# jcjones/ct-mapreduce

Measured on AMD Instinct MI355X. Metric: certificates/sec whole-node + achieved HBM GB/s, 100M-entry synthetic CT batch, higher is better.
Workload: dtype u8

## Files before the change

ct_mapreduce_amd/csrc/ctmr_engine.hip:

```cpp
#include <hip/hip_runtime.h>
#include <dlfcn.h>
#include <rccl/rccl.h>

#include <algorithm>
#include <atomic>
#include <chrono>
#include <condition_variable>
#include <deque>
#include <system_error>
#include <thread>
#include <cmath>
#include <cstdarg>
#include <cstdio>
#include <cstdlib>
#include <cstring>
#include <map>
#include <mutex>
#include <set>
#include <string>
#include <unordered_map>
#include <vector>

#include "host_keys.h"
#include "kernels.h"
// ... 161 lines not shown
  unsigned long long* issuer_counts = nullptr;
  uint32_t epoch = 0;
  bool pairs_dirty = false;
  int known_order = CTMR_KNOWN_ORDER_ANY;
  uint32_t max_issuers = 0;
  uint8_t* d_issuer_valid = nullptr;
  uint32_t* d_canon = nullptr;
  std::vector<IssuerRec> issuers;
  std::unordered_map<std::string, uint32_t> id_to_canon;
  uint8_t* d_idb_der = nullptr;
  size_t idb_cap = 0, idb_used = 0;
  uint64_t* d_idb_off = nullptr;
  uint32_t* d_idb_len = nullptr;
  unsigned long long* d_idb_ht = nullptr;
  uint32_t idb_ht_size = 0;
  std::vector<unsigned long long> h_idb_ht;
  std::unordered_map<std::string, uint32_t> der_to_idx;
  bool auto_register = true;
  int chain0_mode = CTMR_CHAIN0_EXACT;
  bool strict_ext = true;
  bool strict_strings = true;
  bool strict_spki = true;
  bool strict_leaf = true;
  uint64_t meta_precheck_n = 0;
  const uint32_t* meta_precheck_ent = nullptr;
  std::unordered_map<unsigned long long, uint32_t> qh_first;
  std::vector<std::string> pending_issuers;
  unsigned long long* d_pend = nullptr;
  uint32_t* d_unreg = nullptr;
  unsigned long long* d_dcount = nullptr;
  MetaSlot* d_meta_slots = nullptr;
  uint64_t n_meta_slots = 0;
  uint8_t* d_meta_arena = nullptr;
  unsigned long long* d_meta_refs = nullptr;
  uint64_t meta_arena_cap = 0;
  std::vector<uint32_t*> meta_hour_pages;
  uint32_t** d_meta_hour_pages = nullptr;
  unsigned long long* d_mcount = nullptr;
  uint64_t meta_n = 0;
  uint32_t meta_epoch = 0;
  unsigned long long* d_bloom = nullptr;
  uint64_t bloom_words = 0;
  bool bloom_owned = false;
  uint64_t bloom_round_ref0 = ~0ull;
  bool last_meta_valid = false;
  uint64_t last_meta_items = 0;
  bool last_is_view = false;
  size_t last_o_start = 0, last_o_end = 0;
  FilterDev* d_filter = nullptr;
  FilterDev h_filter{};
  DevStats* d_stats = nullptr;
  uint32_t* d_result = nullptr;
  unsigned long long* d_count = nullptr;
  void* d_scratch[28] = {};
  size_t scratch_cap[28] = {};
  RoundCtx rd;
  uint64_t last_n = 0, last_n_new = 0;
  size_t last_o_off = 0, last_o_new = 0;
  hipEvent_t ev[8] = {};
  std::vector<uint64_t> h_rel;
  std::map<std::string, std::set<std::string>> hstore;
  std::map<std::string, int64_t> expiry;
  std::unordered_map<uint32_t, uint64_t> host_issuer_counts;
};

namespace {

enum { SC_RECORDS = 0, SC_SLOTID, SC_BLKNEW, SC_BLKBASE, SC_ENT, SC_STAGE_A, SC_STAGE_B, SC_MISC, SC_PEM, SC_PEMOFF, SC_TMP, SC_VIEW, SC_ISS_A, SC_ISS_B, SC_ISS_C, SC_META, SC_ITEMS,
       SC_XSTAGE, SC_XWCNT, SC_XCNT, SC_XBASE, SC_XSLOT, SC_XL,
       SC_NFX,
       SC_KEYPOS,
       SC_PEMBLK,
       SC_PEMINFO
       };
constexpr uint32_t UNREG_CAP = 16384;

int fail(const ctmr_engine* e, int code, const char* fmt, ...) {
  char buf[512];
  va_list ap;
  va_start(ap, fmt);
  vsnprintf(buf, sizeof buf, fmt, ap);
  va_end(ap);
  if (e) {
    std::lock_guard<std::mutex> g(e->err_mu);
    e->err = buf;
  }
  return code;
}

#define HIPCHK(e, call)                                                                   \
  do {                                                                                    \
    hipError_t _r = (call);                                                               \
    if (_r != hipSuccess)                                                                 \
      return fail(e, _r == hipErrorOutOfMemory ? CTMR_E_NOMEM : CTMR_E_HIP, "%s: %s", #call, \
                  hipGetErrorString(_r));                                                 \
  } while (0)

int ensure(ctmr_engine* e, int which, size_t bytes) {
  if (e->scratch_cap[which] >= bytes) return CTMR_OK;
  if (e->d_scratch[which]) {
    HIPCHK(e, hipStreamSynchronize(e->stream));
    HIPCHK(e, hipFree(e->d_scratch[which]));
    e->d_scratch[which] = nullptr;
    e->scratch_cap[which] = 0;
  }
  size_t cap = bytes + bytes / 8 + 256;
  HIPCHK(e, hipMalloc(&e->d_scratch[which], cap));
  e->scratch_cap[which] = cap;
  return CTMR_OK;
}

struct DevMem {
  void* p = nullptr;
  DevMem() = default;
  DevMem(const DevMem&) = delete;
  DevMem& operator=(const DevMem&) = delete;
  ~DevMem() { if (p) (void)hipFree(p); }
  hipError_t alloc(size_t bytes) {
    if (p) (void)hipFree(p);
    p = nullptr;
    const hipError_t r = hipMalloc(&p, bytes);
    if (r != hipSuccess) {
      (void)hipGetLastError();
      p = nullptr;
    }
    return r;
// ... 332 lines not shown
```

ct_mapreduce_amd/csrc/engine/map.inc:

```

int ctmr_set_filter(ctmr_engine* e, const char* filter, size_t len, int log_expired, int64_t now) {
  if (!e || (len && !filter)) return CTMR_E_INVAL;
  std::lock_guard<std::mutex> g(e->mu);
  HIPCHK(e, hipSetDevice(e->device));
  FilterDev f;
  memset(&f, 0, sizeof f);
  f.active = len != 0;
  f.log_expired = log_expired != 0;
  f.now = now;
  f.strict_spki = e->strict_spki ? 1u : 0u;
  f.strict_strings = e->strict_strings ? 1u : 0u;
  f.strict_ext = e->strict_ext ? 1u : 0u;
  size_t s = 0;
  uint32_t nw = 0;
  for (;;) {
    size_t t = s;
    while (t < len && filter[t] != ',') t++;
    const size_t pl = t - s;
    if (f.n_pieces >= 64 || nw + (pl + 3) / 4 > 1024)
      return fail(e, CTMR_E_INVAL, "issuerCNFilter too large (max 64 pieces / 4096 bytes)");
    f.piece_len[f.n_pieces] = (uint32_t)pl;
    f.piece_word[f.n_pieces] = nw;
    memcpy((uint8_t*)(f.words + nw), filter + s, pl);
    nw += (uint32_t)((pl + 3) / 4);
    f.n_pieces++;
    if (t >= len) break;
    s = t + 1;
  }
  e->h_filter = f;
  return upload_filter(e);
}

static int launch_map(ctmr_engine* e, const uint8_t* d_payload, const uint64_t* d_offsets,
                      const uint32_t* d_issuer_idx, const uint8_t* d_entry_type, uint64_t n,
                      ctmr_record* d_records, bool optimistic_new, const InsertArgs* fuse = nullptr,
                      const uint64_t* d_ends = nullptr, uint64_t limit = 0, int mode = XM_LOCAL,
                      const XchgArgs* xchg = nullptr, uint64_t first = 0) {
  MapArgs ma;
  ma.optimistic_new = optimistic_new ? 1u : 0u;
  ma.ends = d_ends; ma.limit = limit;
  ma.meta_loc = nullptr;
  if (e->cfg.collect_meta) {
    int mr;
    if ((mr = ensure(e, SC_META, (first + n) * 8))) return mr;
    ma.meta_loc = (uint2*)e->d_scratch[SC_META] + first;
    e->meta_n = first + n;
    e->last_meta_valid = false;
  }
  ma.payload = d_payload; ma.offsets = d_offsets; ma.issuer_idx = d_issuer_idx;
  ma.entry_type = d_entry_type; ma.records = d_records; ma.issuer_valid = e->d_issuer_valid;
  ma.filt = e->d_filter; ma.n = n; ma.n_issuers = (uint32_t)e->issuers.size();
  ma.certs_per_tile = 0; ma.lds_bytes = 0;
  ma.keypos = nullptr;
  if (e->strict_spki && n) {
    int kr;
    if ((kr = ensure(e, SC_KEYPOS, (first + n) * 8))) return kr;
    ma.keypos = (unsigned long long*)e->d_scratch[SC_KEYPOS] + first;
  }
  uint32_t variant = e->cfg.map_variant ? e->cfg.map_variant : 15;
  e->meta_precheck_n = 0;
  if (variant == 15 && !fuse) variant = 13;
  const dim3 grid((unsigned)((n + 63) / 64));
#ifdef CTMR_SWEEP
  static const size_t extra_lds = getenv("CTMR_EXTRA_LDS") ? (size_t)atoi(getenv("CTMR_EXTRA_LDS")) : 0;
#else
  constexpr size_t extra_lds = 0;
#endif
  const bool strict = e->strict_strings || e->strict_ext;
  if (variant == 15) {
    MetaCheck mc{};
    XchgArgs xa{};
    if (xchg) xa = *xchg;
    bool meta = false;
    if (e->cfg.collect_meta && e->d_meta_slots) {
      mc.slots = e->d_meta_slots; mc.mask = e->n_meta_slots - 1; mc.arena = e->d_meta_arena;
      mc.hour_pages = e->d_meta_hour_pages; mc.n_hour_pages = e->d_meta_hour_pages ? (uint32_t)e->meta_hour_pages.size() : 0u;
      mc.refs = e->d_meta_refs; mc.n_refs = e->max_issuers;
      mc.enabled = 1;
      meta = true;
      e->meta_precheck_n = first + n;
      e->meta_precheck_ent = fuse->ent - first;
    }
#define CTMR_LAUNCH_FUSED(META, MODE)                                                                                        \
  do {                                                                                                                       \
    if (strict)                                                                                                              \
      hipLaunchKernelGGL((k_map_fused<WIN_CH_STRICT, META, MODE, true>), grid, dim3(64),                                     \
                         WinGeo<WIN_CH_STRICT>::LDS_BYTES + extra_lds, e->stream, ma, *fuse, mc, xa);                        \
    else                                                                                                                     \
      hipLaunchKernelGGL((k_map_fused<WIN_CH_FAST, META, MODE, false>), grid, dim3(64),                                      \
                         WinGeo<WIN_CH_FAST>::LDS_BYTES + extra_lds, e->stream, ma, *fuse, mc, xa);                          \
  } while (0)
    if (mode == XM_OWNER) { if (meta) CTMR_LAUNCH_FUSED(true, XM_OWNER); else CTMR_LAUNCH_FUSED(false, XM_OWNER); }
    else if (mode == XM_BLOOM) { if (meta) CTMR_LAUNCH_FUSED(true, XM_BLOOM); else CTMR_LAUNCH_FUSED(false, XM_BLOOM); }
    else { if (meta) CTMR_LAUNCH_FUSED(true, XM_LOCAL); else CTMR_LAUNCH_FUSED(false, XM_LOCAL); }
#undef CTMR_LAUNCH_FUSED
  } else if (variant == 13) {
    if (strict) hipLaunchKernelGGL((k_map_winc<WIN_CH_STRICT, true>), grid, dim3(64), WinGeo<WIN_CH_STRICT>::LDS_BYTES + extra_lds, e->stream, ma);
    else hipLaunchKernelGGL((k_map_winc<WIN_CH_FAST, false>), grid, dim3(64), WinGeo<WIN_CH_FAST>::LDS_BYTES + extra_lds, e->stream, ma);
#ifdef CTMR_SWEEP
  } else if (variant == 2) {
    hipLaunchKernelGGL(k_map_direct, dim3((unsigned)((n + 255) / 256)), dim3(256), 0, e->stream, ma);
  } else if (variant == 1 && !d_ends) {
    uint32_t C = e->cfg.certs_per_tile ? e->cfg.certs_per_tile : 32;
    if (C > 64) C = 64;
    uint32_t lds = e->cfg.lds_tile_bytes ? e->cfg.lds_tile_bytes : 65536;
    if (lds > 160 * 1024) lds = 160 * 1024;
    ma.certs_per_tile = C; ma.lds_bytes = lds;
    if (!e->tile_attr_set) {
      HIPCHK(e, hipFuncSetAttribute((const void*)k_map_tile, hipFuncAttributeMaxDynamicSharedMemorySize, 160 * 1024));
      e->tile_attr_set = true;
    }
    hipLaunchKernelGGL(k_map_tile, dim3((unsigned)((n + C - 1) / C)), dim3(64), lds, e->stream, ma);
#endif
  } else {
    return fail(e, CTMR_E_INVAL, "map_variant %u is not built into this library", variant);
  }
  return CTMR_OK;
}

static bool round_fused(const ctmr_engine* e) { return e->cfg.map_variant == 0 || e->cfg.map_variant == 15; }

static void round_insert_args(ctmr_engine* e, const RoundCtx& rc, InsertArgs& ia) {
  ia.records = rc.d_records; ia.payload = rc.d_payload; ia.offsets = rc.d_offsets; ia.ends = rc.d_ends; ia.canon = e->d_canon;
  ia.t = e->tbl(); ia.ref0 = rc.ref0; ia.slot_id = (uint32_t*)e->d_scratch[SC_SLOTID];
  ia.ent = (uint32_t*)e->d_scratch[SC_ENT]; ia.n = rc.n; ia.stats = e->d_stats; ia.ord_base = rc.ord_base;
  ia.keypos = (const unsigned long long*)e->d_scratch[SC_KEYPOS]; ia.stage = nullptr; ia.bloom = nullptr; ia.bloom_wmask = 0;
}

static int round_prepare(ctmr_engine* e, RoundCtx& rc) {
  HIPCHK(e, hipSetDevice(e->device));
  e->rd.valid = false;
  const uint64_t n = rc.n;
  if (n >= 0xfffffff0ull) return fail(e, CTMR_E_INVAL, "batch too large (n < 2^32-16)");
  if (((uintptr_t)rc.d_payload & 15) != 0) return fail(e, CTMR_E_INVAL, "payload must be 16-byte aligned");
  int r;
  if (!rc.d_records) {
    if ((r = ensure(e, SC_RECORDS, n * sizeof(ctmr_record)))) return r;
    rc.d_records = (ctmr_record*)e->d_scratch[SC_RECORDS];
  }
  const uint64_t nb = (n + 1023) / 1024;
  if ((r = ensure(e, SC_SLOTID, n * 4))) return r;
  if ((r = ensure(e, SC_ENT, n * 4))) return r;
  if ((r = ensure(e, SC_BLKNEW, nb * 4))) return r;
  if ((r = ensure(e, SC_BLKBASE, nb * 8))) return r;
  if (e->strict_spki && n && (r = ensure(e, SC_KEYPOS, n * 8))) return r;
  if (e->cfg.collect_meta && (r = ensure(e, SC_META, n * 8))) return r;
  if ((r = ensure_capacity(e, n, true))) return r;
  rc.ref0 = e->arena_used;
  e->arena_used += n;
  e->epoch++;
  e->pairs_dirty = true;
  HIPCHK(e, hipMemsetAsync(e->d_stats, 0, 2 * sizeof(DevStats), e->stream));
  const bool fused = round_fused(e);
  if (!fused && rc.mode == XM_OWNER) return fail(e, CTMR_E_INVAL, "the owner-computes exchange needs the fused map kernel (map_variant 0 / 15)");
  if (rc.mode == XM_LOCAL && fused && e->d_bloom) {
    rc.mode = XM_BLOOM;
  }
  if (rc.mode == XM_BLOOM && !e->d_bloom) return fail(e, CTMR_E_INVAL, "ctmr_bloom_config has not been called");
  return CTMR_OK;
}

static int round_launch_range(ctmr_engine* e, RoundCtx& rc, const XchgArgs* xchg, uint64_t lo, uint64_t hi) {
  const uint64_t n = hi - lo;
  if (!n) return CTMR_OK;
  const bool prof = e->cfg.profile != 0;
  int r;
  InsertArgs ia;
  round_insert_args(e, rc, ia);
  ia.records += lo; ia.offsets += lo; ia.slot_id += lo; ia.ent += lo; ia.n = n; ia.ref0 += lo; ia.ord_base += (uint32_t)lo;
  if (ia.ends) ia.ends += lo;
  if (ia.keypos) ia.keypos += lo;
  const bool fused = round_fused(e);
  XchgArgs xa{};
  if (xchg) xa = *xchg;
  if (xa.stage) xa.stage += lo;
  if (xa.wave_cnt) xa.wave_cnt += (lo / 64) * MAX_WORLD;
  if (rc.mode == XM_BLOOM) {
    xa.bloom = e->d_bloom;
    xa.bloom_wmask = e->bloom_words - 1;
  }
  if (prof && lo == 0) HIPCHK(e, hipEventRecord(e->ev[0], e->stream));
  const int kmode = !fused ? XM_LOCAL : (rc.mode == XM_OWNER && rc.world == 1) ? XM_LOCAL : rc.mode;
  if ((r = launch_map(e, rc.d_payload, rc.d_offsets + lo, rc.d_issuer_idx + lo, rc.d_entry_type ? rc.d_entry_type + lo : nullptr, n,
                      rc.d_records + lo, true, fused ? &ia : nullptr, rc.d_ends ? rc.d_ends + lo : nullptr,
                      rc.blob_bytes + CTMR_PAYLOAD_PAD, kmode, &xa, lo)))
    return r;
  if (prof && hi == rc.n) HIPCHK(e, hipEventRecord(e->ev[1], e->stream));
  if (!fused) hipLaunchKernelGGL(k_insert, dim3((unsigned)((n + 255) / 256)), dim3(256), 0, e->stream, ia);
  if (e->strict_spki) {
    ia.stage = (kmode == XM_OWNER) ? xa.stage : nullptr;
    ia.bloom = (rc.mode == XM_BLOOM && fused) ? xa.bloom : nullptr;
    ia.bloom_wmask = xa.bloom_wmask;
    hipLaunchKernelGGL(k_ec_resolve<true>, dim3((unsigned)((n + EC_PER_BLOCK - 1) / EC_PER_BLOCK)), dim3(256), 0, e->stream, ia, rc.d_records + lo);
    hipLaunchKernelGGL(k_ec_resolve<false>, dim3((unsigned)((n + EC_PER_BLOCK - 1) / EC_PER_BLOCK)), dim3(256), 0, e->stream, ia, rc.d_records + lo);
  }
  hipLaunchKernelGGL(k_insert2, dim3((unsigned)((n + INSERT2_PER_BLOCK - 1) / INSERT2_PER_BLOCK)), dim3(256), 0, e->stream, ia, rc.d_records + lo);
  if (!fused && rc.mode == XM_BLOOM)
    hipLaunchKernelGGL(k_bloom_add, dim3((unsigned)((n + 255) / 256)), dim3(256), 0, e->stream, ia, e->d_bloom, e->bloom_words - 1);
  if (prof && hi == rc.n) HIPCHK(e, hipEventRecord(e->ev[2], e->stream));
  return CTMR_OK;
}

static int round_begin(ctmr_engine* e, RoundCtx& rc, const XchgArgs* xchg) {
  int r;
  if ((r = round_prepare(e, rc))) return r;
  return round_launch_range(e, rc, xchg, 0, rc.n);
}

static void round_compact(ctmr_engine* e, const RoundCtx& rc) {
  const uint64_t nb = (rc.n + 1023) / 1024;
  uint32_t* d_blk_new = (uint32_t*)e->d_scratch[SC_BLKNEW];
  uint64_t* d_blk_base = (uint64_t*)e->d_scratch[SC_BLKBASE];
  hipLaunchKernelGGL(k_scan_blocks, dim3(1), dim3(1024), 0, e->stream, d_blk_new, nb, d_blk_base);
  hipLaunchKernelGGL(k_compact, dim3((unsigned)nb), dim3(256), 0, e->stream, (const ctmr_record*)rc.d_records,
                     (const uint32_t*)e->d_scratch[SC_ENT], rc.n, (const uint64_t*)d_blk_base, rc.d_new_idx);
}

static int round_resolve(ctmr_engine* e, RoundCtx& rc, bool compact_now) {
  const bool prof = e->cfg.profile != 0;
  const uint64_t nb = (rc.n + 1023) / 1024;
  ResolveArgs ra;
  ra.ent = (uint32_t*)e->d_scratch[SC_ENT]; ra.issuer_counts = e->issuer_counts; ra.stats = e->d_stats;
  ra.blk_new = (uint32_t*)e->d_scratch[SC_BLKNEW]; ra.n = rc.n;
  hipLaunchKernelGGL(k_resolve, dim3((unsigned)(nb < 512 ? nb : 512)), dim3(1024), 0, e->stream, ra, nb);
  if (prof) HIPCHK(e, hipEventRecord(e->ev[3], e->stream));
  rc.compacted = false;
  if (compact_now && rc.d_new_idx) {
    round_compact(e, rc);
    rc.compacted = true;
  }
  if (prof) HIPCHK(e, hipEventRecord(e->ev[4], e->stream));
  return CTMR_OK;
}

static int round_collect(ctmr_engine* e, RoundCtx& rc) {
  const uint64_t n = rc.n;
  uint32_t* d_ent = (uint32_t*)e->d_scratch[SC_ENT];
  uint32_t* d_blk_new = (uint32_t*)e->d_scratch[SC_BLKNEW];
  DevStats both[2];
  uint64_t ends[2] = {0, rc.blob_bytes};
  HIPCHK(e, hipMemcpyAsync(both, e->d_stats, sizeof both, hipMemcpyDeviceToHost, e->stream));
// ... 184 lines not shown
```

ct_mapreduce_amd/csrc/kernels/reduce.h:

```cpp
#pragma once
#include "keyrec.h"
#include "map.h"

namespace ctmr {

#define AGENT __HIP_MEMORY_SCOPE_AGENT

__device__ __forceinline__ unsigned long long ld_agent(const unsigned long long* p) {
  return __hip_atomic_load(p, __ATOMIC_RELAXED, AGENT);
}
__device__ __forceinline__ void st_agent(unsigned long long* p, unsigned long long v) {
  __hip_atomic_store(p, v, __ATOMIC_RELAXED, AGENT);
}

__device__ __forceinline__ bool cell_equals(const KeyCell* c, unsigned long long meta, const unsigned long long s[5]) {
  bool eq = (ld_agent(&c->meta) & ~CELL_SHADOW) == meta;
#pragma unroll
  for (int k = 0; k < 5; k++) eq = eq && ld_agent(&c->s[k]) == s[k];
  return eq;
}
__device__ __forceinline__ void cell_write(KeyCell* c, unsigned long long meta, const unsigned long long s[5], uint32_t ord) {
  uint4* q = (uint4*)c;
  q[0] = make_uint4((uint32_t)meta, (uint32_t)(meta >> 32), (uint32_t)s[0], (uint32_t)(s[0] >> 32));
  q[1] = make_uint4((uint32_t)s[1], (uint32_t)(s[1] >> 32), (uint32_t)s[2], (uint32_t)(s[2] >> 32));
  q[2] = make_uint4((uint32_t)s[3], (uint32_t)(s[3] >> 32), (uint32_t)s[4], (uint32_t)(s[4] >> 32));
  q[3] = make_uint4(ord, 0u, 0u, 0u);
}

__device__ __forceinline__ uint32_t index_upsert(const Table& t, unsigned long long meta, const unsigned long long s[5],
                                                 unsigned long long my_ref, bool insert, bool* created,
                                                 unsigned long long* holder = nullptr) {
  const unsigned long long h = key_hash(meta, s);
  const unsigned long long mine = idx_word(h, my_ref);
  uint64_t j = h & t.mask;
  *created = false;
  for (uint64_t probes = 0; probes <= t.mask; probes++) {
    unsigned long long w = ld_agent(&t.index[j]);
    if (w == 0ull) {
      if (!insert) return SID_NONE;
      const unsigned long long old = atomicCAS(&t.index[j], 0ull, mine);
      if (old == 0ull) {
        *created = true;
        if (holder) *holder = mine;
        return (uint32_t)j;
      }
      w = old;
    }
    if (w != IDX_TOMB && idx_same_tag(w, h) && cell_equals(t.arena + (w & REF_MASK), meta, s)) {
      if (holder) *holder = w;
      return (uint32_t)j;
    }
    j = probe_next(j, probes, t.mask);
  }
  return SID_FULL;
}

struct InsertArgs {
  const ctmr_record* records;
  const uint8_t* payload;
  const uint64_t* offsets;
  const uint64_t* ends;
  const uint32_t* canon;
  Table t;
  unsigned long long ref0;
  uint32_t* slot_id;
  uint32_t* ent;
  uint64_t n;
  DevStats* stats;
  uint32_t ord_base;
  const unsigned long long* keypos;
  KeyRec32* stage;
  unsigned long long* bloom;
  uint64_t bloom_wmask;
};

enum : uint32_t {
  ES_NONE = 0,
  ES_CLAIMED = 1,
  ES_DEFER = 2,
  ES_DUP = 3,
  ES_HOST = 4,
  ES_FULL = 5,
  ES_REMOTE = 6,
  ES_PENDING = 7
};
constexpr uint32_t ENT_KEY_PENDING = 0x80u;
__device__ __forceinline__ uint32_t ent_pack(uint32_t status, uint32_t state, uint32_t canon) {
  return (status & 7u) | (state << 3) | (canon << 8);
}
__device__ __forceinline__ uint32_t ent_state(uint32_t e) { return (e >> 3) & 7u; }
__device__ __forceinline__ bool ent_is_new(uint32_t e) {
  const uint32_t st = ent_state(e);
  return (st == ES_CLAIMED) | (st == ES_DEFER) | (st == ES_REMOTE);
}
__device__ __forceinline__ void mark_dup(uint32_t* ent, ctmr_record* records, uint32_t loser) {
  ((uint8_t*)(ent + loser))[0] = (uint8_t)(CTMR_ST_PASS | (ES_DUP << 3));
  uint8_t* fl = (uint8_t*)(records + loser) + 1;
  *fl = (uint8_t)(*fl & ~CTMR_FL_WAS_UNKNOWN);
}

__device__ __forceinline__ uint32_t serial_content_off(const GlobalReader& r, uint32_t L) {
  bool ok = true;
  uint32_t tag, cs, ce;
  rd_hdr(r, L, 0, L, ok, tag, cs, ce);
  rd_hdr(r, L, cs, L, ok, tag, cs, ce);
  uint32_t q = cs;
  if ((r.ld4(q) & 0xffu) == 0xa0u) {
    rd_hdr<false>(r, L, q, L, ok, tag, cs, ce);
    rd_hdr(r, L, cs, L, ok, tag, cs, ce);
    q = ce;
  }
  rd_hdr(r, L, q, L, ok, tag, cs, ce);
  return cs;
}

__device__ __forceinline__ void record_key(const InsertArgs& a, uint64_t i, const uint4& r0,
                                           const uint4& r1, unsigned long long s[5]) {
  const uint32_t slen = r0.x >> 16;
  s[0] = (unsigned long long)r0.w | ((unsigned long long)r1.x << 32);
  s[1] = (unsigned long long)r1.y | ((unsigned long long)r1.z << 32);
  s[2] = (unsigned long long)r1.w;
  s[3] = 0;
  s[4] = 0;
  if (slen > 20) {
    uint64_t lo, hi;
    cert_range(a.offsets, a.ends, i, lo, hi);
    GlobalReader g{(const uint32_t*)a.payload, lo};
    const uint32_t so = serial_content_off(g, (uint32_t)(hi - lo));
    uint32_t x[5] = {0, 0, 0, 0, 0};
#pragma unroll
    for (int k = 0; k < 5; k++) {
      const uint32_t pos = 20u + 4u * k;
      if (pos < slen) {
        const uint32_t rem = slen - pos;
        const uint32_t v = g.ld4(so + pos);
        x[k] = rem >= 4 ? v : (v & (0xffffffffu >> (8 * (4 - rem))));
      }
    }
    s[2] |= (unsigned long long)x[0] << 32;
    s[3] = (unsigned long long)x[1] | ((unsigned long long)x[2] << 32);
    s[4] = (unsigned long long)x[3] | ((unsigned long long)x[4] << 32);
  }
}

__device__ __forceinline__ uint32_t insert_probe_h(const InsertArgs& a, uint64_t i, unsigned long long meta,
                                                   const unsigned long long s[5], unsigned long long h) {
  const unsigned long long mine = idx_word(h, a.ref0 + i);
  uint64_t j = h & a.t.mask;
  for (uint64_t probes = 0; probes <= a.t.mask; probes++) {
    const unsigned long long old = atomicCAS(&a.t.index[j], 0ull, mine);
    if (old == 0ull) return ES_CLAIMED;
// ... 27 lines not shown

__device__ __forceinline__ void store_cells_wave(KeyCell* cells, uint64_t n_left, uint4* img, uint32_t lane, bool keyed,
                                                 unsigned long long meta, const unsigned long long s[5], uint32_t ord) {
  uint4* my = img + lane * 4;
  const unsigned long long m = keyed ? meta : 0ull;
  my[0] = make_uint4((uint32_t)m, (uint32_t)(m >> 32), (uint32_t)s[0], (uint32_t)(s[0] >> 32));
  my[1] = make_uint4((uint32_t)s[1], (uint32_t)(s[1] >> 32), (uint32_t)s[2], (uint32_t)(s[2] >> 32));
  my[2] = make_uint4((uint32_t)s[3], (uint32_t)(s[3] >> 32), (uint32_t)s[4], (uint32_t)(s[4] >> 32));
  my[3] = make_uint4(ord, 0u, 0u, 0u);
  __builtin_amdgcn_wave_barrier();
  const uint32_t nvec = n_left >= 64 ? 256u : (uint32_t)n_left * 4u;
  uint4* out = (uint4*)cells;
#pragma unroll
  for (int r = 0; r < 4; r++)
    if (64u * r + lane < nvec) out[64 * r + lane] = img[64 * r + lane];
}

__global__ void __launch_bounds__(256) k_insert(InsertArgs a) {
  __shared__ __attribute__((aligned(16))) uint4 img[4][64 * 4];
  const uint64_t i = (uint64_t)blockIdx.x * 256 + threadIdx.x;
  const uint32_t lane = threadIdx.x & 63, wv = threadIdx.x >> 6;
  uint32_t state = ES_NONE, status = CTMR_ST__COUNT, canon = 0;
  unsigned long long meta = 0ull, s[5] = {0ull, 0ull, 0ull, 0ull, 0ull};
  bool keyed = false;
  if (i < a.n) {
    const uint4* rp = (const uint4*)(a.records + i);
    const uint4 r0 = rp[0];
    status = r0.x & 0xffu;
    const bool pending = ((r0.x >> 8) & FL_KEY_PENDING) != 0u;
    uint32_t fl_out = (r0.x >> 8) & 0xffu & ~FL_KEY_PENDING;
    if (status == CTMR_ST_PASS) {
      canon = a.canon[r0.z];
      const uint4 r1 = rp[1];
      const uint32_t slen = r0.x >> 16;
      if (pending && slen <= CTMR_MAX_SERIAL) {
        state = ES_PENDING;
        record_key(a, i, r0, r1, s);
        meta = key_meta((int32_t)r0.y, canon, slen);
      } else {
        state = insert_probe(a, i, r0, r1, canon, meta, s);
      }
      keyed = slen <= CTMR_MAX_SERIAL;
      if (state != ES_CLAIMED && state != ES_DEFER && state != ES_PENDING) fl_out &= ~(uint32_t)CTMR_FL_WAS_UNKNOWN;
    }
    if (fl_out != ((r0.x >> 8) & 0xffu)) ((uint8_t*)(a.records + i))[1] = (uint8_t)fl_out;
    a.ent[i] = ent_pack(status, state, canon) | (pending ? ENT_KEY_PENDING : 0u);
    const unsigned long long mp = __ballot(pending);
    if (mp && lane == (uint32_t)(__ffsll((long long)mp) - 1) && ld_agent(&a.stats->n_pending) == 0ull) {
      st_agent(&a.stats->n_pending, 1ull);
      st_agent(&a.stats->n_pending_other, 1ull);
    }
  }
  const uint64_t first = (uint64_t)blockIdx.x * 256 + 64u * wv;
  if (first < a.n)
    store_cells_wave(a.t.arena + a.ref0 + first, a.n - first, img[wv], lane, keyed, meta, s, a.ord_base + (uint32_t)i);
}

__device__ __forceinline__ void mark_dup_ord(const InsertArgs& a, ctmr_record* records, uint32_t loser_ord) {
  const uint32_t li = loser_ord - a.ord_base;
  if ((uint64_t)li < a.n) mark_dup(a.ent, records, li);
}

__device__ __forceinline__ bool settle_order(const InsertArgs& a, ctmr_record* records, uint32_t sid, unsigned long long h,
                                             unsigned long long my_ref, uint32_t ord) {
  unsigned long long w = ld_agent(&a.t.index[sid]);
  for (;;) {
    const unsigned long long href = w & REF_MASK;
    if (href == my_ref) return true;
    if (href < a.ref0) return false;
    const uint32_t hord = __hip_atomic_load(&a.t.arena[href].ord, __ATOMIC_RELAXED, AGENT);
    if (hord < ord) return false;
    const unsigned long long old = atomicCAS(&a.t.index[sid], w, idx_word(h, my_ref));
    if (old == w) {
      mark_dup_ord(a, records, hord);
      return true;
    }
    w = old;
  }
}

__device__ __forceinline__ void insert2_one(const InsertArgs& a, ctmr_record* records, uint64_t i, uint32_t e) {
  uint32_t sid = a.slot_id[i];
  const uint4* rp = (const uint4*)(a.records + i);
  const uint4 r0 = rp[0], r1 = rp[1];
  unsigned long long s[5];
  record_key(a, i, r0, r1, s);
  const unsigned long long meta = key_meta((int32_t)r0.y, e >> 8, r0.x >> 16);
  const unsigned long long h = key_hash(meta, s);
  const uint32_t ord = a.ord_base + (uint32_t)i;
  const unsigned long long my_ref = a.ref0 + i;
  const unsigned long long w = ld_agent(&a.t.index[sid]);
  if (!cell_equals(a.t.arena + (w & REF_MASK), meta, s)) {
    bool created;
    unsigned long long holder = 0ull;
    sid = index_upsert(a.t, meta, s, my_ref, true, &created, &holder);
    if (sid == SID_FULL) {
      ((uint8_t*)(a.ent + i))[0] = (uint8_t)(CTMR_ST_PASS | (ES_FULL << 3));
      return;
    }
    if (created) return;
    if ((holder & REF_MASK) < a.ref0) {
      mark_dup(a.ent, records, (uint32_t)i);
      return;
    }
  }
  if (!settle_order(a, records, sid, h, my_ref, ord)) mark_dup(a.ent, records, (uint32_t)i);
}

constexpr uint32_t INSERT2_PER_BLOCK = 1024;
__global__ void __launch_bounds__(256) k_insert2(InsertArgs a, ctmr_record* records) {
  const uint64_t i0 = (uint64_t)blockIdx.x * INSERT2_PER_BLOCK + threadIdx.x * 4u;
  if (i0 >= a.n) return;
  uint32_t e[4] = {0u, 0u, 0u, 0u};
  if (i0 + 4 <= a.n) {
    const uint4 v = *(const uint4*)(a.ent + i0);
    e[0] = v.x; e[1] = v.y; e[2] = v.z; e[3] = v.w;
  } else {
    for (uint32_t k = 0; i0 + k < a.n; k++) e[k] = a.ent[i0 + k];
  }
  uint32_t todo = (ent_state(e[0]) == ES_DEFER ? 1u : 0u) | (ent_state(e[1]) == ES_DEFER ? 2u : 0u) |
                  (ent_state(e[2]) == ES_DEFER ? 4u : 0u) | (ent_state(e[3]) == ES_DEFER ? 8u : 0u);
  while (todo) {
    const uint32_t k = (uint32_t)__builtin_ctz(todo);
    todo &= todo - 1u;
    const uint32_t ek = k == 0u ? e[0] : k == 1u ? e[1] : k == 2u ? e[2] : e[3];
    insert2_one(a, records, i0 + k, ek);
  }
}

template <int WCH, bool META, int MODE, bool STRICT = false>
__global__ void __launch_bounds__(64) k_map_fused(MapArgs a, InsertArgs ia, MetaCheck mc, XchgArgs xa) {
  const uint64_t first = (uint64_t)blockIdx.x * 64;
  const uint32_t lane = threadIdx.x;
  const uint64_t i = first + lane;
  const bool live = i < a.n;
  const uint64_t limit = map_limit(a);
  uint64_t lo = 0, hi = 0;
  if (live) cert_range(a.offsets, a.ends, i, lo, hi);
  EntryIn in{CTMR_NO_ISSUER, 0u, false, false};
  uint32_t canon = 0;
  if (live) {
    in = load_entry_in(a, i);
    canon = in.iss_in_range ? ia.canon[in.iss] : 0u;
  }
  unsigned long long dn_ref = 0, crl_ref = 0;
  const uint32_t* hour_row = nullptr;
  if constexpr (META) {
    if (live && mc.enabled && in.iss_in_range) {
      if (canon < mc.n_refs) {
        dn_ref = mc.refs[canon];
        crl_ref = mc.refs[mc.n_refs + canon];
      }
      if (canon / META_HOUR_PAGE < mc.n_hour_pages)
        hour_row = mc.hour_pages[canon / META_HOUR_PAGE] + (uint64_t)(canon % META_HOUR_PAGE) * (META_HOUR_BITS / 32);
    }
  }
  const WaveBuf wb = wave_buf(a.payload, limit, lo);
  const uint32_t lrel = wave_rel(wb, lo, live);
  const uint32_t w_me = lrel == REL_NONE ? REL_NONE : ((lrel + WinGeo<WCH>::SKIP) & ~3u);
  U16t hd16{0u, 0u, 0u, 0u};
  bool hd_ok = false;
  if constexpr (WinGeo<WCH>::SKIP != 0u) {
    hd_ok = live & (lo + 16ull <= limit);
    hd16 = *(const U16t*)(a.payload + (hd_ok ? lo : 0ull));
  }
  coop_fill<WCH, false>(wb, w_me, lane);
  uint4 o0 = make_uint4(0, 0, 0, 0), o1 = o0;
  unsigned long long kmeta = 0ull, ks[5] = {0ull, 0ull, 0ull, 0ull, 0ull};
  bool keyed = false;
  uint32_t rem_owner = KEY_NO_OWNER;
  bool rem_long = false;
  uint4 k0 = make_uint4(0, 0, 0, 0), k1 = k0;
  unsigned long long keypos = 0ull;
  bool pending = false;
  if (live) {
    using Hook = typename std::conditional<META, MetaHook, NoRefillHook>::type;
    WinReaderS<WCH, Hook> r{{{(const uint32_t*)a.payload, lo, limit, (uint32_t*)(smem + win_off<WCH>(lane)),
                              lrel == REL_NONE ? (int32_t)0x80000000 : (int32_t)(w_me - lrel), wb, lrel}},
                            lrel == REL_NONE ? 0xffffffffu : 0u, {0u, 0u, 0u, 0u, 0u, 0u, 0u, 0u}, 0x80000000u};
    if constexpr (WinGeo<WCH>::SKIP != 0u) {
      r.hd[0] = hd16.a; r.hd[1] = hd16.b; r.hd[2] = hd16.c; r.hd[3] = hd16.d;
      r.hd_ok = hd_ok;
    }
    if constexpr (META) {
      r.hook.mc = mc;
      r.hook.canon = canon;
      r.hook.dn_ref = dn_ref;
      r.hook.dn_seen = false;
    }
    uint2 ml = make_uint2(META_NONE, META_NONE);
    map_one<STRICT>(r, hi - lo, i, a, in, o0, o1, &ml, &keypos);
    if (r.missed()) {
      GlobalReader g{(const uint32_t*)a.payload, lo};
      map_one<STRICT>(g, hi - lo, i, a, in, o0, o1, nullptr, &keypos);
    }
    pending = keypos != 0ull;
    o0.x &= ~(FL_KEY_PENDING << 8);
    const uint32_t status = o0.x & 0xffu;
    uint32_t state = ES_NONE;
    MetaTail mt;
    bool meta_try = false;
    if constexpr (META) {
      meta_try = mc.enabled && status == CTMR_ST_PASS && !r.missed() && ml.x != META_NONE && ml.x != META_HOST && r.hook.dn_seen;
      if (meta_try)
        mt = meta_tail_issue(mc, crl_ref, hour_row, (int32_t)o0.y, ml.y, r.win, r.grel, r.part ? 0u : WinReader<WCH>::WBYTES - 8u);
    }
    if (status == CTMR_ST_PASS) {
      const uint32_t slen = o0.x >> 16;
      if (slen > CTMR_MAX_SERIAL) {
        state = ES_HOST;
      } else {
        unsigned long long* const s = ks;
        record_key(ia, i, o0, o1, s);
        const unsigned long long meta = kmeta = key_meta((int32_t)o0.y, canon, slen);
        keyed = true;
        const unsigned long long h = key_hash(meta, s);
        bool mine = true;
        if constexpr (MODE == XM_OWNER) {
          rem_owner = key_owner_h(h, xa.world);
          mine = rem_owner == xa.rank;
        }
        if (mine) {
#ifdef CTMR_EXP_NO_PROBE
          state = ES_CLAIMED;
#else
          state = pending ? (uint32_t)ES_PENDING : insert_probe_h(ia, i, meta, s, h);
#endif
        } else {
          state = ES_REMOTE;
          rem_long = slen > 20u;
          k0 = make_uint4((uint32_t)meta, (uint32_t)(meta >> 32), (uint32_t)s[0], (uint32_t)(s[0] >> 32));
          k1 = make_uint4((uint32_t)s[1], (uint32_t)(s[1] >> 32), (uint32_t)s[2], ia.ord_base + (uint32_t)i);
        }
        if constexpr (MODE == XM_BLOOM) {
          if (state == ES_CLAIMED || state == ES_DEFER) {
            uint64_t word;
            unsigned long long bits;
            bloom_pos(h, xa.bloom_wmask, word, bits);
            atomicOr(&xa.bloom[word], bits);
          }
        }
      }
      if (state != ES_CLAIMED && state != ES_DEFER && state != ES_REMOTE && state != ES_PENDING)
        o0.x &= ~((uint32_t)CTMR_FL_WAS_UNKNOWN << 8);
    }
    uint32_t e = ent_pack(status, state, canon) | (pending ? ENT_KEY_PENDING : 0u);
    if constexpr (META) {
      const bool seen = meta_try && meta_tail_finish(mc, canon, mt, (int32_t)o0.y, r.win);
      e |= seen ? 0u : ENT_META_UNSEEN;
    }
    ia.ent[i] = e;
  }
  store_records_wave(a, first, live, o0, o1);
  __builtin_amdgcn_wave_barrier();
  if (first < a.n)
    store_cells_wave(ia.t.arena + ia.ref0 + first, a.n - first, (uint4*)smem, lane, keyed, kmeta, ks, ia.ord_base + (uint32_t)i);
  {
    const unsigned long long mp = __ballot(pending);
    if (mp && lane == 0 && ld_agent(&ia.stats->n_pending) == 0ull) st_agent(&ia.stats->n_pending, 1ull);
    const unsigned long long mo = __ballot(pending && ((keypos >> 32) & 7ull) != 1ull);
    if (mo && lane == 0 && ld_agent(&ia.stats->n_pending_other) == 0ull) st_agent(&ia.stats->n_pending_other, 1ull);
    if constexpr (MODE != XM_OWNER) {
      if (pending) a.keypos[i] = keypos;
    }
  }
  if constexpr (MODE == XM_OWNER) {
    const bool rem = rem_owner != KEY_NO_OWNER && rem_owner != xa.rank && !rem_long;
    const unsigned long long lt = (1ull << lane) - 1ull;
    uint32_t pos = 0, before = 0, mine_cnt = 0;
    for (uint32_t o = 0; o < xa.world; o++) {
      const unsigned long long m = __ballot(rem && rem_owner == o);
      const uint32_t c = (uint32_t)__popcll(m);
      if (rem && rem_owner == o) pos = before + (uint32_t)__popcll(m & lt);
      if (lane == o) mine_cnt = c;
      before += c;
    }
    if (rem) {
      uint4* out = (uint4*)(xa.stage + first + pos);
      out[0] = k0;
      out[1] = k1;
    }
    if (pending) a.keypos[i] = keypos | (rem ? (1ull << 38) | ((unsigned long long)pos << 39) : 0ull);
    if (lane < MAX_WORLD) xa.wave_cnt[(uint64_t)blockIdx.x * MAX_WORLD + lane] = (uint8_t)mine_cnt;
    const unsigned long long ml = __ballot(rem_owner != KEY_NO_OWNER && rem_owner != xa.rank && rem_long);
    if (ml && lane == 0) atomicAdd(&ia.stats->n_xl, (unsigned long long)__popcll(ml));
  }
}


template <class C>
__device__ __forceinline__ bool ec_point_bits(const uint32_t* words, unsigned long long xbit) {
  uint32_t x[C::NL], y[C::NL];
  fe_load_bits<C>(words, xbit, x);
  fe_load_bits<C>(words, xbit + 8ull * C::BYTES, y);
  return ec_equation<C>(x, y);
}

constexpr uint32_t EC_PER_BLOCK = 1024;
template <bool P256>
__global__ void __launch_bounds__(256) k_ec_resolve(InsertArgs a, ctmr_record* records) {
  __shared__ uint16_t list[EC_PER_BLOCK];
  __shared__ uint32_t n_list;
  if ((P256 ? a.stats->n_pending : a.stats->n_pending_other) == 0ull) return;
  const uint64_t blk0 = (uint64_t)blockIdx.x * EC_PER_BLOCK;
  if (threadIdx.x == 0) n_list = 0u;
  __syncthreads();
  {
    const uint64_t i0 = blk0 + threadIdx.x * 4u;
    uint32_t e[4] = {0u, 0u, 0u, 0u};
    if (i0 + 4 <= a.n) {
      const uint4 v = *(const uint4*)(a.ent + i0);
      e[0] = v.x; e[1] = v.y; e[2] = v.z; e[3] = v.w;
    } else {
      for (uint32_t k = 0; i0 + k < a.n; k++) e[k] = a.ent[i0 + k];
    }
#pragma unroll
    for (uint32_t k = 0; k < 4; k++)
      if ((e[k] & ENT_KEY_PENDING) && ((((uint32_t)(a.keypos[i0 + k] >> 32) & 7u) == 1u) == P256))
        list[atomicAdd(&n_list, 1u)] = (uint16_t)(threadIdx.x * 4u + k);
  }
  __syncthreads();
  const uint32_t cnt = n_list;
  for (uint32_t base = 0; base < cnt; base += 256u) {
    const uint32_t t = base + threadIdx.x;
    if (t < cnt) {
      const uint64_t i = blk0 + list[t];
      const uint32_t e = a.ent[i];
      const unsigned long long kp = a.keypos[i];
      uint64_t lo, hi;
      cert_range(a.offsets, a.ends, i, lo, hi);
      const uint32_t pos = (uint32_t)kp, curve = (uint32_t)(kp >> 32) & 7u, shift = (uint32_t)(kp >> 35) & 7u;
      const unsigned long long xbit = 8ull * (lo + pos) - shift;
      uint4* rp = (uint4*)(records + i);
      const uint4 r0 = rp[0], r1 = rp[1];
      bool good;
      if constexpr (P256) {
        good = ec_point_bits<CurveP256>((const uint32_t*)a.payload, xbit);
      } else {
        switch (curve) {
          case 2u: good = ec_point_bits<CurveP384>((const uint32_t*)a.payload, xbit); break;
          case 3u: good = ec_point_bits<CurveP521>((const uint32_t*)a.payload, xbit); break;
          case 4u: good = ec_point_bits<CurveP224>((const uint32_t*)a.payload, xbit); break;
          default: good = ec_point_bits<CurveP192>((const uint32_t*)a.payload, xbit); break;
        }
      }
      if (!good) {
        const uint32_t stn = (r0.x & 0xffu) == CTMR_ST_ENTRY_DECODE_ERROR ? (uint32_t)CTMR_ST_ENTRY_DECODE_ERROR : (uint32_t)CTMR_ST_PARSE_ERROR;
        rp[0] = make_uint4(stn | (((r0.x >> 8) & CTMR_FL_PRECERT) << 8), 0u, r0.z, 0u);
        rp[1] = make_uint4(0u, 0u, 0u, 0u);
        if ((kp >> 38) & 1ull) {
          a.stage[(i & ~63ull) + ((kp >> 39) & 63ull)].meta = 0ull;
        } else if (ent_state(e) == ES_REMOTE) {
          atomicAdd(&a.stats->n_xl, ~0ull);
        }
        a.ent[i] = ent_pack(stn, ES_NONE, e >> 8);
      } else if (ent_state(e) != ES_PENDING) {
        a.ent[i] = e & ~ENT_KEY_PENDING;
      } else {
        unsigned long long s[5];
        record_key(a, i, r0, r1, s);
        const unsigned long long meta = key_meta((int32_t)r0.y, e >> 8, r0.x >> 16);
        const unsigned long long h = key_hash(meta, s);
        const uint32_t state = insert_probe_h(a, i, meta, s, h);
        if (state != ES_CLAIMED && state != ES_DEFER) {
          ((uint8_t*)(records + i))[1] = (uint8_t)((r0.x >> 8) & ~CTMR_FL_WAS_UNKNOWN);
        } else if (a.bloom) {
          uint64_t word;
          unsigned long long bits;
          bloom_pos(h, a.bloom_wmask, word, bits);
          atomicOr(&a.bloom[word], bits);
        }
        a.ent[i] = (e & ~(ENT_KEY_PENDING | (7u << 3))) | (state << 3);
      }
    }
  }
}

__device__ __forceinline__ void wave_agg_add(bool active, uint32_t key, unsigned long long* arr) {
  unsigned long long todo = __ballot(active);
  while (todo) {
    const int leader = __ffsll((long long)todo) - 1;
    const uint32_t k = __shfl(key, leader);
    const unsigned long long same = __ballot(active && key == k) & todo;
    if ((int)(threadIdx.x & 63) == leader) atomicAdd(&arr[k], (unsigned long long)__popcll(same));
    todo &= ~same;
  }
}

__device__ __forceinline__ bool pair_add(PairSlot* pairs, uint64_t pmask, unsigned long long key,
                                         long long delta) {
  uint64_t j = mixk(key) & pmask;
  for (uint64_t probes = 0; probes <= pmask; probes++) {
    unsigned long long k = ld_agent(&pairs[j].key);
    if (k == 0ull) {
      const unsigned long long old = atomicCAS(&pairs[j].key, 0ull, key);
      k = old == 0ull ? key : old;
    }
    if (k == key) {
      atomicAdd(&pairs[j].count, (unsigned long long)delta);
      return true;
    }
    j = (j + 1) & pmask;
  }
  return false;
}

struct ResolveArgs {
  const uint32_t* ent;
  unsigned long long* issuer_counts;
  DevStats* stats;
  uint32_t* blk_new;
  uint64_t n;
};

constexpr uint32_t RES_LDS_ISSUERS = 4096;

// ... 227 lines not shown
```

Before: 2.519 billion.

## Add region-sorted hash insert path and defer bitmask for second-pass insert

Adds an optional mode, enabled by the CTMR_REGION_SLOTS environment variable, where the fused map kernel records each key's home slot instead of probing the hash table. A count/scan/scatter pass then groups entries by table region before a separate insert kernel runs, so probes hit nearby table memory. Separately, the kernels now write a per-64-entry deferred bitmask, and k_insert2 builds a shared-memory list from that bitmask instead of scanning every ent word. The region path adds extra kernels, scratch buffers and an extra read of staged cells. The bitmask adds a write in the default path.

Result: no change. 2.504 billion (-0.6%).

```diff
diff --git a/ct_mapreduce_amd/csrc/ctmr_engine.hip b/ct_mapreduce_amd/csrc/ctmr_engine.hip
--- a/ct_mapreduce_amd/csrc/ctmr_engine.hip
+++ b/ct_mapreduce_amd/csrc/ctmr_engine.hip
@@ -237,8 +237,8 @@
   DevStats* d_stats = nullptr;
   uint32_t* d_result = nullptr;
   unsigned long long* d_count = nullptr;
-  void* d_scratch[28] = {};
-  size_t scratch_cap[28] = {};
+  void* d_scratch[32] = {};
+  size_t scratch_cap[32] = {};
   RoundCtx rd;
   uint64_t last_n = 0, last_n_new = 0;
   size_t last_o_off = 0, last_o_new = 0;
@@ -256,7 +256,11 @@
        SC_NFX,
        SC_KEYPOS,
        SC_PEMBLK,
-       SC_PEMINFO
+       SC_PEMINFO,
+       SC_DEFER,
+       SC_RGCNT,
+       SC_RGSUM,
+       SC_RGLIST
        };
 constexpr uint32_t UNREG_CAP = 16384;
 
diff --git a/ct_mapreduce_amd/csrc/engine/map.inc b/ct_mapreduce_amd/csrc/engine/map.inc
--- a/ct_mapreduce_amd/csrc/engine/map.inc
+++ b/ct_mapreduce_amd/csrc/engine/map.inc
@@ -31,6 +31,26 @@
   return upload_filter(e);
 }
 
+static bool round_region_insert(const ctmr_engine* e, int kmode) {
+  const char* v = getenv("CTMR_REGION_SLOTS");
+  if (!v || strtoull(v, nullptr, 0) == 0) return false;
+  return (e->cfg.map_variant == 0 || e->cfg.map_variant == 15) && kmode == XM_LOCAL && !(e->cfg.collect_meta && e->d_meta_slots);
+}
+
+constexpr uint64_t REGION_SLOTS = 1ull << 23;
+static void round_region_geo(const ctmr_engine* e, uint32_t& shift, uint32_t& n_regions) {
+  uint64_t slots = REGION_SLOTS;
+  if (const char* v = getenv("CTMR_REGION_SLOTS")) {
+    const uint64_t x = strtoull(v, nullptr, 0);
+    if (x && !(x & (x - 1))) slots = x;
+  }
+  shift = 0;
+  while ((1ull << shift) < slots) shift++;
+  while ((e->nslots >> shift) > REGION_MAX) shift++;
+  n_regions = (uint32_t)(e->nslots >> shift);
+  if (n_regions == 0) n_regions = 1;
+}
+
 static int launch_map(ctmr_engine* e, const uint8_t* d_payload, const uint64_t* d_offsets,
                       const uint32_t* d_issuer_idx, const uint8_t* d_entry_type, uint64_t n,
                       ctmr_record* d_records, bool optimistic_new, const InsertArgs* fuse = nullptr,
@@ -81,18 +101,20 @@
       e->meta_precheck_n = first + n;
       e->meta_precheck_ent = fuse->ent - first;
     }
-#define CTMR_LAUNCH_FUSED(META, MODE)                                                                                        \
+#define CTMR_LAUNCH_FUSED(META, MODE, REGION)                                                                                \
   do {                                                                                                                       \
     if (strict)                                                                                                              \
-      hipLaunchKernelGGL((k_map_fused<WIN_CH_STRICT, META, MODE, true>), grid, dim3(64),                                     \
+      hipLaunchKernelGGL((k_map_fused<WIN_CH_STRICT, META, MODE, true, REGION>), grid, dim3(64),                             \
                          WinGeo<WIN_CH_STRICT>::LDS_BYTES + extra_lds, e->stream, ma, *fuse, mc, xa);                        \
     else                                                                                                                     \
-      hipLaunchKernelGGL((k_map_fused<WIN_CH_FAST, META, MODE, false>), grid, dim3(64),                                      \
+      hipLaunchKernelGGL((k_map_fused<WIN_CH_FAST, META, MODE, false, REGION>), grid, dim3(64),                              \
                          WinGeo<WIN_CH_FAST>::LDS_BYTES + extra_lds, e->stream, ma, *fuse, mc, xa);                          \
   } while (0)
-    if (mode == XM_OWNER) { if (meta) CTMR_LAUNCH_FUSED(true, XM_OWNER); else CTMR_LAUNCH_FUSED(false, XM_OWNER); }
-    else if (mode == XM_BLOOM) { if (meta) CTMR_LAUNCH_FUSED(true, XM_BLOOM); else CTMR_LAUNCH_FUSED(false, XM_BLOOM); }
-    else { if (meta) CTMR_LAUNCH_FUSED(true, XM_LOCAL); else CTMR_LAUNCH_FUSED(false, XM_LOCAL); }
+    if (mode == XM_OWNER) { if (meta) CTMR_LAUNCH_FUSED(true, XM_OWNER, false); else CTMR_LAUNCH_FUSED(false, XM_OWNER, false); }
+    else if (mode == XM_BLOOM) { if (meta) CTMR_LAUNCH_FUSED(true, XM_BLOOM, false); else CTMR_LAUNCH_FUSED(false, XM_BLOOM, false); }
+    else if (meta) CTMR_LAUNCH_FUSED(true, XM_LOCAL, false);
+    else if (round_region_insert(e, mode)) CTMR_LAUNCH_FUSED(false, XM_LOCAL, true);
+    else CTMR_LAUNCH_FUSED(false, XM_LOCAL, false);
 #undef CTMR_LAUNCH_FUSED
   } else if (variant == 13) {
     if (strict) hipLaunchKernelGGL((k_map_winc<WIN_CH_STRICT, true>), grid, dim3(64), WinGeo<WIN_CH_STRICT>::LDS_BYTES + extra_lds, e->stream, ma);
@@ -120,11 +142,38 @@
 
 static bool round_fused(const ctmr_engine* e) { return e->cfg.map_variant == 0 || e->cfg.map_variant == 15; }
 
+static int round_insert_regions(ctmr_engine* e, const InsertArgs& ia, ctmr_record* d_records) {
+  const uint64_t n = ia.n;
+  const dim3 grid((unsigned)((n + 255) / 256));
+  RegionArgs g;
+  round_region_geo(e, g.shift, g.n_regions);
+  if (g.n_regions == 1) {
+    hipLaunchKernelGGL(k_insert_regions, grid, dim3(256), 0, e->stream, ia, d_records, (const uint32_t*)nullptr,
+                       (const unsigned long long*)nullptr);
+    return CTMR_OK;
+  }
+  g.home = ia.slot_id; g.n = n;
+  g.n_tiles = (n + REGION_TILE - 1) / REGION_TILE;
+  const uint64_t n_cnt = (uint64_t)g.n_regions * g.n_tiles + 1;
+  int r;
+  if ((r = ensure(e, SC_RGCNT, n_cnt * 8))) return r;
+  if ((r = ensure(e, SC_RGLIST, n * 4))) return r;
+  g.cnt = (unsigned long long*)e->d_scratch[SC_RGCNT];
+  g.list = (uint32_t*)e->d_scratch[SC_RGLIST];
+  hipLaunchKernelGGL(k_region_count, dim3((unsigned)g.n_tiles), dim3(256), 0, e->stream, g);
+  if ((r = scan_u64(e, (uint64_t*)g.cnt, n_cnt, false, SC_RGSUM))) return r;
+  hipLaunchKernelGGL(k_region_scatter, dim3((unsigned)g.n_tiles), dim3(256), 0, e->stream, g);
+  hipLaunchKernelGGL(k_insert_regions, grid, dim3(256), 0, e->stream, ia, d_records, (const uint32_t*)g.list,
+                     (const unsigned long long*)(g.cnt + n_cnt - 1));
+  return CTMR_OK;
+}
+
 static void round_insert_args(ctmr_engine* e, const RoundCtx& rc, InsertArgs& ia) {
   ia.records = rc.d_records; ia.payload = rc.d_payload; ia.offsets = rc.d_offsets; ia.ends = rc.d_ends; ia.canon = e->d_canon;
   ia.t = e->tbl(); ia.ref0 = rc.ref0; ia.slot_id = (uint32_t*)e->d_scratch[SC_SLOTID];
   ia.ent = (uint32_t*)e->d_scratch[SC_ENT]; ia.n = rc.n; ia.stats = e->d_stats; ia.ord_base = rc.ord_base;
   ia.keypos = (const unsigned long long*)e->d_scratch[SC_KEYPOS]; ia.stage = nullptr; ia.bloom = nullptr; ia.bloom_wmask = 0;
+  ia.defer = (unsigned long long*)e->d_scratch[SC_DEFER];
 }
 
 static int round_prepare(ctmr_engine* e, RoundCtx& rc) {
@@ -141,6 +190,7 @@
   const uint64_t nb = (n + 1023) / 1024;
   if ((r = ensure(e, SC_SLOTID, n * 4))) return r;
   if ((r = ensure(e, SC_ENT, n * 4))) return r;
+  if ((r = ensure(e, SC_DEFER, (n + 63) / 64 * 8))) return r;
   if ((r = ensure(e, SC_BLKNEW, nb * 4))) return r;
   if ((r = ensure(e, SC_BLKBASE, nb * 8))) return r;
   if (e->strict_spki && n && (r = ensure(e, SC_KEYPOS, n * 8))) return r;
@@ -167,7 +217,7 @@
   int r;
   InsertArgs ia;
   round_insert_args(e, rc, ia);
-  ia.records += lo; ia.offsets += lo; ia.slot_id += lo; ia.ent += lo; ia.n = n; ia.ref0 += lo; ia.ord_base += (uint32_t)lo;
+  ia.records += lo; ia.offsets += lo; ia.slot_id += lo; ia.ent += lo; ia.defer += lo / 64; ia.n = n; ia.ref0 += lo; ia.ord_base += (uint32_t)lo;
   if (ia.ends) ia.ends += lo;
   if (ia.keypos) ia.keypos += lo;
   const bool fused = round_fused(e);
@@ -187,6 +237,7 @@
     return r;
   if (prof && hi == rc.n) HIPCHK(e, hipEventRecord(e->ev[1], e->stream));
   if (!fused) hipLaunchKernelGGL(k_insert, dim3((unsigned)((n + 255) / 256)), dim3(256), 0, e->stream, ia);
+  else if (round_region_insert(e, kmode) && (r = round_insert_regions(e, ia, rc.d_records + lo))) return r;
   if (e->strict_spki) {
     ia.stage = (kmode == XM_OWNER) ? xa.stage : nullptr;
     ia.bloom = (rc.mode == XM_BLOOM && fused) ? xa.bloom : nullptr;
diff --git a/ct_mapreduce_amd/csrc/kernels/reduce.h b/ct_mapreduce_amd/csrc/kernels/reduce.h
--- a/ct_mapreduce_amd/csrc/kernels/reduce.h
+++ b/ct_mapreduce_amd/csrc/kernels/reduce.h
@@ -72,6 +72,7 @@
   KeyRec32* stage;
   unsigned long long* bloom;
   uint64_t bloom_wmask;
+  unsigned long long* defer;
 };
 
 enum : uint32_t {
@@ -97,6 +98,10 @@
   ((uint8_t*)(ent + loser))[0] = (uint8_t)(CTMR_ST_PASS | (ES_DUP << 3));
   uint8_t* fl = (uint8_t*)(records + loser) + 1;
   *fl = (uint8_t)(*fl & ~CTMR_FL_WAS_UNKNOWN);
+}
+
+__device__ __forceinline__ void defer_mark(const InsertArgs& a, uint64_t i) {
+  atomicOr(&a.defer[i >> 6], 1ull << (i & 63u));
 }
 
 __device__ __forceinline__ uint32_t serial_content_off(const GlobalReader& r, uint32_t L) {
@@ -230,8 +235,11 @@
     }
   }
   const uint64_t first = (uint64_t)blockIdx.x * 256 + 64u * wv;
-  if (first < a.n)
+  const unsigned long long md = __ballot(state == ES_DEFER);
+  if (first < a.n) {
+    if (lane == 0) a.defer[first >> 6] = md;
     store_cells_wave(a.t.arena + a.ref0 + first, a.n - first, img[wv], lane, keyed, meta, s, a.ord_base + (uint32_t)i);
+  }
 }
 
 __device__ __forceinline__ void mark_dup_ord(const InsertArgs& a, ctmr_record* records, uint32_t loser_ord) {
@@ -285,28 +293,31 @@
   if (!settle_order(a, records, sid, h, my_ref, ord)) mark_dup(a.ent, records, (uint32_t)i);
 }
 
-constexpr uint32_t INSERT2_PER_BLOCK = 1024;
+constexpr uint32_t INSERT2_WORDS = 256, INSERT2_PER_BLOCK = 64 * INSERT2_WORDS;
 __global__ void __launch_bounds__(256) k_insert2(InsertArgs a, ctmr_record* records) {
-  const uint64_t i0 = (uint64_t)blockIdx.x * INSERT2_PER_BLOCK + threadIdx.x * 4u;
-  if (i0 >= a.n) return;
-  uint32_t e[4] = {0u, 0u, 0u, 0u};
-  if (i0 + 4 <= a.n) {
-    const uint4 v = *(const uint4*)(a.ent + i0);
-    e[0] = v.x; e[1] = v.y; e[2] = v.z; e[3] = v.w;
-  } else {
-    for (uint32_t k = 0; i0 + k < a.n; k++) e[k] = a.ent[i0 + k];
-  }
-  uint32_t todo = (ent_state(e[0]) == ES_DEFER ? 1u : 0u) | (ent_state(e[1]) == ES_DEFER ? 2u : 0u) |
-                  (ent_state(e[2]) == ES_DEFER ? 4u : 0u) | (ent_state(e[3]) == ES_DEFER ? 8u : 0u);
-  while (todo) {
-    const uint32_t k = (uint32_t)__builtin_ctz(todo);
-    todo &= todo - 1u;
-    const uint32_t ek = k == 0u ? e[0] : k == 1u ? e[1] : k == 2u ? e[2] : e[3];
-    insert2_one(a, records, i0 + k, ek);
-  }
-}
-
-template <int WCH, bool META, int MODE, bool STRICT = false>
+  __shared__ uint16_t list[INSERT2_PER_BLOCK];
+  __shared__ uint32_t n_list;
+  const uint64_t blk0 = (uint64_t)blockIdx.x * INSERT2_PER_BLOCK;
+  if (threadIdx.x == 0) n_list = 0u;
+  __syncthreads();
+  const uint64_t w = (uint64_t)blockIdx.x * INSERT2_WORDS + threadIdx.x;
+  unsigned long long m = w * 64u < a.n ? a.defer[w] : 0ull;
+  if (m) {
+    uint32_t at = atomicAdd(&n_list, (uint32_t)__popcll(m));
+    while (m) {
+      list[at++] = (uint16_t)(threadIdx.x * 64u + (uint32_t)__ffsll((long long)m) - 1u);
+      m &= m - 1ull;
+    }
+  }
+  __syncthreads();
+  const uint32_t cnt = n_list;
+  for (uint32_t t = threadIdx.x; t < cnt; t += 256u) {
+    const uint64_t i = blk0 + list[t];
+    insert2_one(a, records, i, a.ent[i]);
+  }
+}
+
+template <int WCH, bool META, int MODE, bool STRICT = false, bool REGION = false>
 __global__ void __launch_bounds__(64) k_map_fused(MapArgs a, InsertArgs ia, MetaCheck mc, XchgArgs xa) {
   const uint64_t first = (uint64_t)blockIdx.x * 64;
   const uint32_t lane = threadIdx.x;
@@ -351,6 +362,8 @@
   uint4 k0 = make_uint4(0, 0, 0, 0), k1 = k0;
   unsigned long long keypos = 0ull;
   bool pending = false;
+  uint32_t home = SID_NONE;
+  bool deferred = false;
   if (live) {
     using Hook = typename std::conditional<META, MetaHook, NoRefillHook>::type;
     WinReaderS<WCH, Hook> r{{{(const uint32_t*)a.payload, lo, limit, (uint32_t*)(smem + win_off<WCH>(lane)),
@@ -402,7 +415,12 @@
 #ifdef CTMR_EXP_NO_PROBE
           state = ES_CLAIMED;
 #else
-          state = pending ? (uint32_t)ES_PENDING : insert_probe_h(ia, i, meta, s, h);
+          if constexpr (REGION) {
+            state = pending ? (uint32_t)ES_PENDING : (uint32_t)ES_CLAIMED;
+            if (!pending) home = (uint32_t)(h & ia.t.mask);
+          } else {
+            state = pending ? (uint32_t)ES_PENDING : insert_probe_h(ia, i, meta, s, h);
+          }
 #endif
         } else {
           state = ES_REMOTE;
@@ -428,6 +446,12 @@
       e |= seen ? 0u : ENT_META_UNSEEN;
     }
     ia.ent[i] = e;
+    if constexpr (REGION) ia.slot_id[i] = home;
+    deferred = state == ES_DEFER;
+  }
+  {
+    const unsigned long long md = __ballot(deferred);
+    if (lane == 0) ia.defer[blockIdx.x] = md;
   }
   store_records_wave(a, first, live, o0, o1);
   __builtin_amdgcn_wave_barrier();
@@ -462,6 +486,83 @@
     if (lane < MAX_WORLD) xa.wave_cnt[(uint64_t)blockIdx.x * MAX_WORLD + lane] = (uint8_t)mine_cnt;
     const unsigned long long ml = __ballot(rem_owner != KEY_NO_OWNER && rem_owner != xa.rank && rem_long);
     if (ml && lane == 0) atomicAdd(&ia.stats->n_xl, (unsigned long long)__popcll(ml));
+  }
+}
+
+constexpr uint32_t REGION_TILE = 4096;
+constexpr uint32_t REGION_MAX = 1024;
+struct RegionArgs {
+  const uint32_t* home;
+  uint64_t n;
+  uint32_t shift;
+  uint32_t n_regions;
+  uint64_t n_tiles;
+  unsigned long long* cnt;
+  uint32_t* list;
+};
+
+template <class F>
+__device__ __forceinline__ void region_tile_each(const RegionArgs& g, F f) {
+  const uint64_t base = (uint64_t)blockIdx.x * REGION_TILE + threadIdx.x * 4u;
+#pragma unroll
+  for (uint32_t p = 0; p < REGION_TILE / 1024u; p++) {
+    const uint64_t i0 = base + p * 1024u;
+    uint32_t v[4] = {SID_NONE, SID_NONE, SID_NONE, SID_NONE};
+    if (i0 + 4 <= g.n) {
+      const uint4 q = *(const uint4*)(g.home + i0);
+      v[0] = q.x; v[1] = q.y; v[2] = q.z; v[3] = q.w;
+    } else {
+      for (uint32_t k = 0; i0 + k < g.n; k++) v[k] = g.home[i0 + k];
+    }
+#pragma unroll
+    for (uint32_t k = 0; k < 4; k++)
+      if (v[k] != SID_NONE) f((uint32_t)(i0 + k), v[k]);
+  }
+}
+
+__global__ void __launch_bounds__(256) k_region_count(RegionArgs g) {
+  __shared__ uint32_t hist[REGION_MAX];
+  for (uint32_t k = threadIdx.x; k < g.n_regions; k += 256u) hist[k] = 0u;
+  __syncthreads();
+  region_tile_each(g, [&](uint32_t, uint32_t slot) { atomicAdd(&hist[slot >> g.shift], 1u); });
+  __syncthreads();
+  for (uint32_t k = threadIdx.x; k < g.n_regions; k += 256u) g.cnt[(uint64_t)k * g.n_tiles + blockIdx.x] = hist[k];
+  if (blockIdx.x == 0 && threadIdx.x == 0) g.cnt[(uint64_t)g.n_regions * g.n_tiles] = 0ull;
+}
+
+__global__ void __launch_bounds__(256) k_region_scatter(RegionArgs g) {
+  __shared__ uint32_t cur[REGION_MAX];
+  for (uint32_t k = threadIdx.x; k < g.n_regions; k += 256u) cur[k] = (uint32_t)g.cnt[(uint64_t)k * g.n_tiles + blockIdx.x];
+  __syncthreads();
+  region_tile_each(g, [&](uint32_t i, uint32_t slot) { g.list[atomicAdd(&cur[slot >> g.shift], 1u)] = i; });
+}
+
+__global__ void __launch_bounds__(256) k_insert_regions(InsertArgs a, ctmr_record* records, const uint32_t* list,
+                                                        const unsigned long long* total) {
+  const uint64_t t = (uint64_t)blockIdx.x * 256 + threadIdx.x;
+  uint64_t i = t;
+  if (list) {
+    if (t >= *total) return;
+    i = list[t];
+  } else if (t >= a.n || a.slot_id[t] == SID_NONE) {
+    return;
+  }
+  const uint4* c = (const uint4*)(a.t.arena + a.ref0 + i);
+  const uint4 c0 = c[0], c1 = c[1], c2 = c[2];
+  const unsigned long long meta = (unsigned long long)c0.x | ((unsigned long long)c0.y << 32);
+  const unsigned long long s[5] = {(unsigned long long)c0.z | ((unsigned long long)c0.w << 32),
+                                   (unsigned long long)c1.x | ((unsigned long long)c1.y << 32),
+                                   (unsigned long long)c1.z | ((unsigned long long)c1.w << 32),
+                                   (unsigned long long)c2.x | ((unsigned long long)c2.y << 32),
+                                   (unsigned long long)c2.z | ((unsigned long long)c2.w << 32)};
+  const uint32_t state = insert_probe_h(a, i, meta, s, key_hash(meta, s));
+  if (state == ES_CLAIMED) return;
+  if (state == ES_DEFER) {
+    ((uint8_t*)(a.ent + i))[0] = (uint8_t)(CTMR_ST_PASS | (ES_DEFER << 3));
+    defer_mark(a, i);
+  } else {
+    mark_dup(a.ent, records, (uint32_t)i);
+    if (state != ES_DUP) ((uint8_t*)(a.ent + i))[0] = (uint8_t)(CTMR_ST_PASS | (state << 3));
   }
 }
 
@@ -540,6 +641,7 @@
         const unsigned long long meta = key_meta((int32_t)r0.y, e >> 8, r0.x >> 16);
         const unsigned long long h = key_hash(meta, s);
         const uint32_t state = insert_probe_h(a, i, meta, s, h);
+        if (state == ES_DEFER) defer_mark(a, i);
         if (state != ES_CLAIMED && state != ES_DEFER) {
           ((uint8_t*)(records + i))[1] = (uint8_t)((r0.x >> 8) & ~CTMR_FL_WAS_UNKNOWN);
         } else if (a.bloom) {
```
